# iyak/RNAelem

Hardware: AMD Instinct MI355X
Metric: train-iter seqs/sec (inside+outside) (higher is better)
Workload: dtype f64; 1 GPU; 10000 synthetic RNAs L=200, pattern ((.*.)), W=50 C=30 min_bpp=1e-4 T2004, x0 lambda=(1,1), one (fn,gr) eval per step; n_seq=10000, seq_len=200, pattern=((.*.)), bpp_filter=cached (computed once at load_batch, 0.1 s incl. plan), n_skipped=0

## Files before the change

rnaelem_amd/csrc/lin_fast.h:

```cpp
#pragma once
#include "lin_rules.h"
#include "plan_rules.h"

namespace elemdp {

#ifndef ELEMDP_UNARY2
#define ELEMDP_UNARY2 1
#endif

constexpr int kCellInD = 10;
constexpr int kCellOutD = 14;
enum : int { CF_POK = 1, CF_LOK = 2, CF_MOK = 4, CF_EOK = 8, CF_DO2 = 16, CF_DOM = 32, CF_CE = 64, CF_CP = 128,
             CF_UP = 64, CF_DOL = 128,
             CF_YL = 1 << 17, CF_YR = 1 << 18, CF_JLAST = 1 << 19,
             CF_USH = 20 };
ELEMDP_HD int fcol(int packed, int byte) { const int c = (packed >> (8 * byte)) & 0xff; return c == 0xff ? -1 : c; }

ELEMDP_HD double cell_in_fetch(const SeqView& q, int d, int i, int k) {
  const int c_here = q.cell(i, d), c_up = (i > 0 && d + 2 <= q.W) ? q.cell(i - 1, d + 2) : c_here;
  const int term = k < 2 ? XT_STACK : k < 4 ? XT_ML : k < 6 ? XT_CLOSE : XT_HP;
  return xw_cell(q, k & 1, term, k < 4 ? c_here : c_up);
}
ELEMDP_HD int cell_in_flags(const ModelView& m, const SeqView& q, int d, int i) {
  const int j = i + d;
// ... 255 lines not shown
  __builtin_amdgcn_sched_barrier(0);
#endif
  const double in1 = in.ldc(ST_1, d, i, c1o, lok && u1), in2 = in.ldc(ST_2, d, i, c2o, lok && u2), inL = LPOST ? 0. : in.ldc(ST_L, d, i, cLo, isloop && uL);
  const double r7 = out.ldc(ST_P, d, i, cPo, pok);
  double op2[kFR], opL[kFR];
  int eR[kFR];
#pragma unroll
  for (int u = 0; u < kFR; ++u) {
    eR[u] = P[4 + u];
    op2[u] = out.ldc(ST_2, dp1, i, fcol(eR[u], 0), u < nRR && do2);
    opL[u] = LPOST ? 0. : out.ldc(ST_L, dp1, i, fcol(eR[u], 1), u < nRR && doL && eR[u] < 0);
  }
#endif
  const double in2z = in2 * invZ, inLz = inL * invZ;
  const bool a2 = do2 && in2 != 0., aL = !LPOST && doL && inL != 0.;
#pragma unroll
  for (int u = 0; u < kFR; ++u)
    if (u < nRR && (a2 || aL)) {
      const int id = (eR[u] >> 16) & 0x7fff;
      const int enr = G[A.fe_r + 2 * id], fr = G[A.fe_r + 2 * id + 1];
      const double w = lin[A.lin_wr + 5 * id + br] * ((fr & 1) ? ews_r : 1.);
      const double t2 = a2 ? op2[u] * w : 0., tL = aL ? opL[u] * w : 0.;
      const double z = fma(t2, in2z, tL * inLz);
      if (SCANM && !fast_scan_stat<MODE, false, true>(sink, FS[id], i - 1, j, yl, yr, jlast, z)) continue;
      if (MODE != OUT_END && !no_prf && z != 0. && br) sink.en(enr + br, z);
      s2 += t2;
      sL += tL;
    }
  double H1 = ph[0], H2 = ph[CS], HP = ph[2 * CS], HL = LPOST ? 0. : ph[3 * CS];
  for (int r = 1; r < nrep; ++r) {
    H1 += ph[r * rstride]; H2 += ph[r * rstride + CS]; HP += ph[r * rstride + 2 * CS];
    if (!LPOST) HL += ph[r * rstride + 3 * CS];
  }
  const double o1 = (in1 != 0.) ? H1 : 0.;
  const double oB = lok ? (mok ? oM : 0.) + o1 : 0.;
  const double o2 = (in2 != 0.) ? o1 + s2 : 0.;
  if (lok && c2o >= 0) out.band[out.cidx(ST_2, d, i, c2o)] = o2;
  double oP = 0.;
  if (inP != 0.) {
    const double t3b = (o2 + H2) * cr[6 + kl], z = t3b * inPz;
    if (MODE == OUT_TRAIN && z != 0.) sink.eh(ehs, cr[13] * z);
    oP = oP1b + t3b + (HP + r7);
  }
  if (pok && cPo >= 0) out.band[out.cidx(ST_P, d, i, cPo)] = oP;
  if (LPOST) return oB;
  double oL = 0.;
  if (inL != 0.) {
    const double t6b = oE * cr[4 + kl], z = t6b * inLz;
    if (MODE == OUT_TRAIN && z != 0.) sink.eh(ehs, cr[11] * z);
    oL = t6b + sL + HL;
  }
  if (cLo >= 0) out.band[out.cidx(ST_L, d, i, cLo)] = oL;
  return oB;
}

ELEMDP_HD double loop_outside_seed_term(double oE, double inP, double inLo, double xw) { return oE * (inP * inLo) * xw; }

template <int kFR, class Sink>
ELEMDP_HD double loop_outside_entry(const int32_t* P, const int32_t* G, int fe_r, const double* wr, const double* parent, double inL,
                                    double HL, double oE, double xhp, double e_hp, bool doL, int br, double ews_r, double invZ, int ehs,
                                    bool no_prf, Sink& sink) {
  if (inL == 0.) return 0.;
  const int nRR = (P[0] >> 8) & 15;
  const double inLz = inL * invZ;
  double sL = 0.;
  if (doL) {
#pragma unroll
    for (int u = 0; u < kFR; ++u)
      if (u < nRR) {
        const int e = P[4 + u], c = fcol(e, 1), id = (e >> 16) & 0x7fff;
        const int enr = G[fe_r + 2 * id], fr = G[fe_r + 2 * id + 1];
        const double w = wr[5 * id + br] * ((fr & 1) ? ews_r : 1.);
        const double tL = (e < 0 && c >= 0) ? parent[c] * w : 0.;
        const double z = tL * inLz;
        if (!no_prf && z != 0. && br) sink.en(enr + br, z);
        sL += tL;
      }
  }
  const double t6b = oE * xhp, z = t6b * inLz;
  if (z != 0.) sink.eh(ehs, e_hp * z);
  return t6b + sL + HL;
}

}
```

rnaelem_amd/csrc/lin_kernels.hip:

```cpp
#include <hip/hip_runtime.h>

#include <algorithm>
#include <cstdio>
#include <cstdlib>
#include <type_traits>

#ifndef ELEMDP_KCI
#define ELEMDP_KCI 2
#endif
#ifndef ELEMDP_LB_IN
#define ELEMDP_LB_IN 4
#endif
#ifndef ELEMDP_LB_IN_FAST
#define ELEMDP_LB_IN_FAST 8
#endif
#ifndef ELEMDP_LB_CYK
#define ELEMDP_LB_CYK 8
#endif
#ifndef ELEMDP_LB_OUT6
#define ELEMDP_LB_OUT6 6
#endif
#ifndef ELEMDP_LB_OUT
#define ELEMDP_LB_OUT 4
#endif
// ... 1616 lines not shown
      }
    }
    hp[slot] = oB;
  }
  __syncthreads();
  if (!(a.dbg & 1) && !(a.dbg & 128) && !(ELEMDP_KO & 8)) {
    const int nA = A.n_ap;
    double* const en_keep = sink.en_;
    for (int w = tid; w < nc * nA; w += kBT) {
      const int c = div_rcp(w, a.rcp_nap), p = w - c * nA;
      if (ci(c) + d <= end_ys) continue;
      if (FAST) {
        const int32_t* PR = G + A.fpr_out + 8 * p;
        const int r0 = PR[0], r1 = PR[1];
        const int tg = (r0 >> 16) & 0xff;
        const bool w1 = pi.merged && (r0 & (4 << 24));
        const int i = ci(c), j = i + d, dmi = dm[c];
        const bool exists = dmi > 0 && dmi < d;
        const bool dead = MASK && exists && !((crfl[c] >> CF_USH) & UB_A);
        if (dead) {
          out.a(d, i, p) = 0.;
        } else if (exists) {
          const bool step = d + 1 <= W && j < L && v.q.unp[j];
          const int nr = step ? (r1 >> 20) & 15 : 0;
          const double a_in = in.a(d, i, p);
          int ce[kFastR];
          double op[kFastR];
#pragma unroll
          for (int u = 0; u < kFastR; ++u) {
            ce[u] = PR[5 + u];
            op[u] = out.lda(d + 1, i, u < nr ? ce[u] & 0xff : p, u < nr);
          }
          double acc = 0.;
          if (a_in != 0.) {
            acc = tg != 0xff ? hp[c * HD + tg] : 0.;
            const double inz = a_in * (w1 ? pi.invZs : pi.invZ);
            const int bj = step ? (int)v.q.seq[j] : 0;
            const double ewj = step ? v.q.ews[j] : 1.;
            double* en = l_en + (w1 ? nt : 0);
#pragma unroll
            for (int u = 0; u < kFastR; ++u)
              if (u < nr) {
                const int id = (ce[u] >> 8) & 0x7fff;
                const double term = op[u] * (v.m.lin[A.lin_wr + 5 * id + bj] * ((G[A.fe_r + 2 * id + 1] & 1) ? ewj : 1.));
                const double z = term * inz;
                if ((MODE == OUT_SCAN || MODE == OUT_END) &&
                    !fast_scan_stat<MODE, false, true>(sink, G[A.fs_out + id], i - 1, j, false, MODE == OUT_END && j == a.ys[v.n], L == j + 1, z))
                  continue;
                if (MODE != OUT_END && !v.m.no_prf && z != 0. && bj) atomicAdd(&en[G[A.fe_r + 2 * id] + bj], z);
                acc += term;
              }
          }
          out.a(d, i, p) = acc;
        }
        continue;
      }
      const int tgt = v.m.ints[A.ap_tgt + p];
      const bool w1 = pi.merged && v.m.ints[A.ap_t + p] == A.shadow;
      sink.en_ = l_en + (w1 ? nt : 0);
      LinOutCtx<LinSink> x{v.m, v.q, in, out, w1 ? pi.invZs : pi.invZ, sink, Constraint{MODE == OUT_END ? a.ys[v.n] : -1, -1, 0}};
      lin_outside_apair<MODE>(x, d, i0 + c, p, tgt >= 0 ? hp[c * HD + tgt] : 0.);
    }
    sink.en_ = en_keep;
  }
  pc.mark<11>();
  if (MODE == OUT_SCAN || MODE == OUT_END) {
    __syncthreads();
    const int p1 = (i0 + nc + d < L) ? i0 + nc + d : L;
    for (int t = tid; t <= p1 - pos_p0; t += kBT) {
      const double v0 = l_pos[t], v1 = l_pos[win + t];
      if (MODE == OUT_SCAN) {
        if (v0 != 0. && pos_p0 + t < L) atomicAdd(&a.pos_start[v.seq_base + pos_p0 + t], v0);
        if (v1 != 0. && pos_p0 + t < L) atomicAdd(&a.pos_inner[v.seq_base + pos_p0 + t], v1);
      } else if (v0 != 0.) {
        atomicAdd(&a.pos_end[v.pos_base + pos_p0 + t], v0);
      }
    }
  }
  if (MODE == OUT_TRAIN || MODE == OUT_SCAN) lflush(a, v, pi, sink, l_en0, kBT, (int)bx);
  pc.mark<12>();
  pc.finish();
}

constexpr int kSeedRows = 8, kSeedDiags = 17, kSeedCap = 256;
static size_t loop_seed_lds(const AutomatonLayout& A) {
  return sizeof(double) * ((size_t)kSeedRows * kSeedDiags * A.n_lane + 2 * kSeedCap) +
         sizeof(int32_t) * (kSeedRows * (kSeedDiags + 1) + kSeedRows + 1 + kLoopColsMax + 4 * kSeedCap + 2 * (size_t)A.n_quad);
}
__global__ __launch_bounds__(kBT) void k4_out_seed(LinArgs a) {
  extern __shared__ double lds[];
  LViews v(a.lay);
  make_lviews(a, blockIdx.y, v);
  if (v.row[4] != 0.) return;
  const AutomatonLayout& A = a.lay;
  const int tid = threadIdx.x, L = v.q.L, W = v.q.W;
  const int i0 = blockIdx.x * kSeedRows, d0 = blockIdx.z * kSeedDiags;
  if (d0 > W || i0 + d0 > L) return;
  const int nrow = (kSeedRows < L - i0 + 1) ? kSeedRows : L - i0 + 1, nd = (kSeedDiags < W - d0 + 1) ? kSeedDiags : W - d0 + 1;
  const int HD = A.n_lane, nq = A.n_quad, rs = v.out.rs[ST_L];
  double* acc = lds;
  double* s_xw = acc + kSeedRows * kSeedDiags * HD;
  int* offs = reinterpret_cast<int*>(s_xw + 2 * kSeedCap);
  int* pre = offs + kSeedRows * (kSeedDiags + 1);
  int* cmap = pre + kSeedRows + 1;
  int* s_row = cmap + kLoopColsMax;
  int* tq = s_row + 4 * kSeedCap;
  for (int t = tid; t < kSeedRows * kSeedDiags * HD; t += kBT) acc[t] = 0.;
  if (tid < kLoopColsMax) cmap[tid] = -1;
  __syncthreads();
  for (int k = tid; k < HD; k += kBT) {
    const int c = fcol(a.ints[A.fp_out + a.ints[A.f_live_out + k] * kFastW + 2], 2);
    if (c >= 0 && c < kLoopColsMax) cmap[c] = k;
  }
  const int32_t* G = v.m.big;
  const double* IB = v.in.band;
  const double* OB = v.out.band;
  const float rcp_nq = 1.0f / (float)(nq > 0 ? nq : 1);
  for (int role = 1; role <= 2; ++role) {
    const int32_t* off = role == 1 ? v.q.by_left_off : v.q.by_right_off;
    const LoopItem* items = role == 1 ? v.q.items_left : v.q.items_right;
    __syncthreads();
    for (int t = tid; t < nrow * (nd + 1); t += kBT) {
      const int r = t / (nd + 1), dd = t - r * (nd + 1), d = d0 + dd;
      offs[r * (kSeedDiags + 1) + dd] = nq > 0 ? off[v.q.cell(i0 + r, d > 0 ? d : 1)] : 0;
    }
    for (int t = tid; t < 2 * nq; t += kBT) tq[t] = G[A.fqc_out + role * 2 * nq + t];
    __syncthreads();
    if (tid == 0) {
      int n = 0;
      for (int r = 0; r < nrow; ++r) { pre[r] = n; n += offs[r * (kSeedDiags + 1) + nd] - offs[r * (kSeedDiags + 1)]; }
      pre[nrow] = n;
    }
    __syncthreads();
    const int n_rec = pre[nrow];
    for (int p0 = 0; p0 < n_rec; p0 += kSeedCap) {
      const int np = (kSeedCap < n_rec - p0) ? kSeedCap : n_rec - p0;
      for (int xs = tid; xs < np; xs += kBT) {
        const int x = p0 + xs;
        int r = 0;
        while (r + 1 < nrow && pre[r + 1] <= x) ++r;
        const int* ro = offs + r * (kSeedDiags + 1);
        const int n = ro[0] + (x - pre[r]);
        int dd = 0;
        while (dd + 1 < nd && ro[dd + 1] <= n) ++dd;
        const int i = i0 + r, d = d0 + dd;
        const bool on = i + d <= L && (v.q.ubits(i, d) & UB_L);
        const LoopItem it = items[n];
        s_row[xs] = (int)v.out.cidx(ST_E, it.j - it.i, it.i, 0);
        s_row[kSeedCap + xs] = (int)v.in.cidx(ST_P, it.l - it.k, it.k, 0);
        s_row[2 * kSeedCap + xs] = (int)(role == 1 ? v.in.cidx(ST_L, it.j - it.l, it.l, 0) : v.in.cidx(ST_L, it.k - it.i, it.i, 0));
        s_row[3 * kSeedCap + xs] = on ? (r * kSeedDiags + dd) * HD : -1;
        s_xw[xs] = lin_weight(v.m.lambda[0], it.tsc);
        s_xw[kSeedCap + xs] = lin_weight(v.m.lambda[1], it.tsc);
      }
      __syncthreads();
      for (int w = tid; w < np * nq; w += kBT) {
        const int xs = div_rcp(w, rcp_nq), t = w - xs * nq;
        const int cell = s_row[3 * kSeedCap + xs];
        const int qa = tq[2 * t], qb = tq[2 * t + 1];
        if (cell < 0 || (qb & (4 << 16))) continue;
        const double x0 = OB[(uint32_t)s_row[xs] + (qa & 0xff)], x1 = IB[(uint32_t)s_row[kSeedCap + xs] + ((qa >> 8) & 0xff)];
        const double x2 = IB[(uint32_t)s_row[2 * kSeedCap + xs] + ((qa >> 16) & 0xff)];
        const double term = loop_outside_seed_term(x0, x1, x2, s_xw[((qb >> 16) & 1) * kSeedCap + xs]);
        if (term != 0.) atomicAdd(&acc[cell + (qb & 0xffff)], term);
      }
      __syncthreads();
    }
  }
  __syncthreads();
  const int run = kSeedRows * rs;
  for (int t = tid; t < nd * run; t += kBT) {
    const int dd = t / run, e = t - dd * run, r = e / rs, c = e - r * rs, d = d0 + dd;
    if (i0 + r + d > L) continue;
    const int k = c < kLoopColsMax ? cmap[c] : -1;
    v.out.band[v.out.cidx(ST_L, d, i0, 0) + e] = k >= 0 ? acc[(r * kSeedDiags + dd) * HD + k] : 0.;
  }
}

static size_t loop_chain_lds(const AutomatonLayout& A) {
  return sizeof(double) * (2 * (size_t)kBT + 5 * (size_t)A.n_wr + 2 * (size_t)A.n_theta + 4) + sizeof(int32_t) * kLoopColsMax * (kLoopProgW + 1);
}
__global__ __launch_bounds__(kBT) void k4_out_loops(LinArgs a) {
  extern __shared__ double lds[];
  LViews v(a.lay);
  make_lviews(a, blockIdx.y, v);
  const LPass pi = lpass(a, v);
  if (pi.skip) return;
  const AutomatonLayout& A = a.lay;
  const int tid = threadIdx.x, L = v.q.L, W = v.q.W, nt = A.n_theta;
  const int rs = v.out.rs[ST_L], R = kBT / rs;
  const int i0 = blockIdx.x * R;
  if (i0 > L) return;
  double* cur = lds;
  double* prev = lds + kBT;
  double* wr = lds + 2 * kBT;
  double* l_en = wr + 5 * A.n_wr;
  int32_t* prog = reinterpret_cast<int32_t*>(l_en + 2 * nt + 4);
  int32_t* pst = prog + kLoopColsMax * kLoopProgW;
  for (int t = tid; t < kLoopColsMax * (kLoopProgW + 1); t += kBT) prog[t] = 0;
  for (int t = tid; t < 5 * A.n_wr; t += kBT) wr[t] = a.lin[A.lin_wr + t];
  for (int t = tid; t < 2 * nt + 4; t += kBT) l_en[t] = 0.;
  cur[tid] = 0.; prev[tid] = 0.;
  __syncthreads();
  for (int k = tid; k < A.n_lane; k += kBT) {
    const int s = a.ints[A.f_live_out + k];
    const int32_t* P = a.ints + A.fp_out + s * kFastW;
    const int c = fcol(P[2], 2);
    if (c >= 0 && c < kLoopColsMax) {
      for (int w = 0; w < kLoopProgW; ++w) prog[c * kLoopProgW + w] = P[w];
      pst[c] = s;
    }
  }
  __syncthreads();
  const int r = tid / rs, c = tid - r * rs, i = i0 + r;
  const int32_t* P = prog + (r < R ? c : 0) * kLoopProgW;
  const int w0 = P[0];
  const bool have = r < R && i <= L && (w0 & 1);
  const bool w1 = pi.merged && pst[r < R ? c : 0] == A.shadow;
  const int kl = (w0 >> 2) & 1, cEo = fcol(P[1], 1), ehs = v.m.lam_same ? 0 : kl;
  const double invZ = w1 ? pi.invZs : pi.invZ;
  LinSink sink;
  sink.world = w1 ? 1 : 0;
  sink.en_ = l_en + (w1 ? nt : 0);
  sink.eh0 = sink.eh1 = 0.;
  const int dmax = (W < L - i0) ? W : L - i0;
  auto cell_on = [&](int d) { return have && d >= 0 && i + d <= L && (v.q.ubits(i, d) & UB_L); };
  bool on_n = cell_on(dmax);
  double inL_n = on_n ? v.in.band[v.in.cidx(ST_L, dmax, i, c)] : 0., HL_n = on_n ? v.out.band[v.out.cidx(ST_L, dmax, i, c)] : 0.;
  for (int d = dmax; d >= 0; --d) {
    double oL = 0.;
    const bool on = on_n;
    const double inL = inL_n, HL = HL_n;
    on_n = cell_on(d - 1);
    inL_n = on_n ? v.in.band[v.in.cidx(ST_L, d - 1, i, c)] : 0.;
    HL_n = on_n ? v.out.band[v.out.cidx(ST_L, d - 1, i, c)] : 0.;
    if (on) {
      if (inL != 0.) {
        const int j = i + d;
        const bool eok = v.q.e_ok(i, d), doL = j < L && d + 1 <= W;
        const int c_up = eok ? v.q.cell(i - 1, d + 2) : v.q.cell(i, d);
        const double oE = (eok && cEo >= 0) ? v.out.band[v.out.cidx(ST_E, d, i, cEo)] : 0.;
        const double xhp = eok ? xw_cell(v.q, kl, XT_HP, c_up) : 0.;
        oL = loop_outside_entry<kFastR>(P, v.m.big, A.fe_r, wr, prev + r * rs, inL, HL, oE, xhp, v.q.e_hp[c_up], doL, j < L ? (int)v.q.seq[j] : 0,
                                        v.q.ews[j < L ? j : L], invZ, ehs, v.m.no_prf != 0, sink);
      }
    }
    cur[tid] = oL;
    __syncthreads();
    double* x = cur; cur = prev; prev = x;
  }
  lflush(a, v, pi, sink, l_en, kBT, (int)blockIdx.x);
}

__global__ __launch_bounds__(kThreads) void k4_combine(LinArgs a, int G) {
  const int g = blockIdx.x;
  if (g >= G) return;
  const int n = a.grp[g];
  double* row = a.seq_out + (size_t)n * a.out_stride;
  if (row[4] != 0.) return;
  const double* zs = a.zs + (size_t)g * 4;
  const int nt = a.lay.n_theta;
  if (a.det) {
    const double* dr = a.det_rows + (size_t)n * a.det_nslot * a.out_stride;
    for (int t = 6 + threadIdx.x; t < 6 + 2 * nt + 4; t += kThreads) {
      double acc = 0.;
      for (int k = 0; k < a.det_nslot; ++k) acc += dr[(size_t)k * a.out_stride + t];
      row[t] = acc;
    }
    __syncthreads();
  }
  const bool positive = a.plans[n].positive != 0;
  const double pa = zs[1] / zs[0], pn = zs[2] / zs[0];
  for (int t = threadIdx.x; t < nt + 2; t += kThreads) {
    double* A = (t < nt) ? &row[6 + t] : &row[6 + 2 * nt + (t - nt)];
    double* B = (t < nt) ? &row[6 + nt + t] : &row[6 + 2 * nt + 2 + (t - nt)];
    const double va = *A, vb = *B;
    if (a.schedule == 1) {
      const double full = pa * va + pn * vb;
      if (a.lik_ratio && !positive) { *A = va; *B = full; }
      else { *A = full; *B = positive ? va : vb; }
    } else if (a.lik_ratio && !positive) {
      *A = vb; *B = va;
    }
  }
}

__device__ __forceinline__ unsigned long long cyk_key(double v) {
  const long long b = __double_as_longlong(v + 0.);
  return (unsigned long long)(b >= 0 ? b : (b ^ 0x7fffffffffffffffLL)) ^ 0x8000000000000000ULL;
}
__device__ __forceinline__ double cyk_unkey(unsigned long long k) {
  const long long b = (long long)(k ^ 0x8000000000000000ULL);
  return __longlong_as_double(b >= 0 ? b : (b ^ 0x7fffffffffffffffLL));
}

__global__ __launch_bounds__(kThreads) void k5_cyk_serial(LinArgs a) {
  __shared__ AutomatonLayout s_lay;
  stage_layout(a, &s_lay, kThreads);
  unsigned bx, by;
  swizzled_block(bx, by);
  LViews v(s_lay);
  make_lviews(a, by, v);
  __syncthreads();
  const int S = a.lay.S, d = a.d;
  if (d > v.q.W) return;
  const int t = bx * kThreads + threadIdx.x;
  if (t >= (v.q.L - d + 1) * S) return;
  const int i = t / S, s = t - i * S;
  TraceView R;
  R.ext = nullptr;
  const Constraint c{a.ys[v.n], a.ye[v.n], 1};
  cyk_target(v.m, v.q, v.in, R, c, d, i, s);
}

template <bool BIG, int KOWN>
__global__ __launch_bounds__(kBT, KOWN <= 2 ? ELEMDP_LB_CYK : 6) void k5_cyk(LinArgs a) {
  extern __shared__ double lds[];

  unsigned bx, by;
  swizzled_block(bx, by);
  LViews v(a.lay);
  make_lviews(a, by, v);
  const AutomatonLayout& A = a.lay;
  const int S = a.lay.S, d = a.d, cpb = a.cpb, tid = threadIdx.x;
  if (d > v.q.W) return;
  const int ncell = v.q.L - d + 1, i0 = bx * cpb;
  if (i0 >= ncell) return;
  const int nc = (cpb < ncell - i0) ? cpb : ncell - i0;
  const int NL = A.n_lane;
  const int CS = cpb * NL;
  const double NEG = ELEMDP_NEG_INF;
  unsigned long long* kb = reinterpret_cast<unsigned long long*>(lds);
  unsigned long long* ke = kb + CS;
  double* st1 = lds + 2 * CS;
// ... 279 lines not shown
    case K4_GENERIC: hipLaunchKernelGGL((k4_in<false, CON>), grid, dim3(kBT), lds, st, a); break;
  }
}
template <int MODE>
static void launch_k4_out(const LinArgs& a, dim3 grid, size_t lds, bool fast, bool big, hipStream_t st) {
  if (MODE == OUT_TRAIN && fast && a.loop_post) {
    const bool l = a.p.blocks != nullptr;
    switch (k4_form(a, lds, 6, fast, big)) {
      case K4_FP2_WAVES:
        if (l) hipLaunchKernelGGL((k4_out<OUT_TRAIN, true, true, 2, true, true, true>), grid, dim3(kBT), lds, st, a);
        else hipLaunchKernelGGL((k4_out<OUT_TRAIN, true, true, 2, true, false, true>), grid, dim3(kBT), lds, st, a);
        return;
      case K4_FP2:
        if (l) hipLaunchKernelGGL((k4_out<OUT_TRAIN, true, true, 2, false, true, true>), grid, dim3(kBT), lds, st, a);
        else hipLaunchKernelGGL((k4_out<OUT_TRAIN, true, true, 2, false, false, true>), grid, dim3(kBT), lds, st, a);
        return;
      default:
        if (l) hipLaunchKernelGGL((k4_out<OUT_TRAIN, true, true, kFastP, false, true, true>), grid, dim3(kBT), lds, st, a);
        else hipLaunchKernelGGL((k4_out<OUT_TRAIN, true, true, kFastP, false, false, true>), grid, dim3(kBT), lds, st, a);
        return;
    }
  }
  if (MODE == OUT_TRAIN && fast && a.p.blocks) {
    switch (k4_form(a, lds, 6, fast, big)) {
      case K4_FP2_WAVES: hipLaunchKernelGGL((k4_out<OUT_TRAIN, true, true, 2, true, true>), grid, dim3(kBT), lds, st, a); return;
      case K4_FP2: hipLaunchKernelGGL((k4_out<OUT_TRAIN, true, true, 2, false, true>), grid, dim3(kBT), lds, st, a); return;
      default: hipLaunchKernelGGL((k4_out<OUT_TRAIN, true, true, kFastP, false, true>), grid, dim3(kBT), lds, st, a); return;
    }
  }
  switch (k4_form(a, lds, 6, fast, big)) {
    case K4_FP2_WAVES: hipLaunchKernelGGL((k4_out<MODE, true, true, 2, true>), grid, dim3(kBT), lds, st, a); break;
    case K4_FP2: hipLaunchKernelGGL((k4_out<MODE, true, true, 2>), grid, dim3(kBT), lds, st, a); break;
    case K4_FAST: hipLaunchKernelGGL((k4_out<MODE, true, true>), grid, dim3(kBT), lds, st, a); break;
    case K4_STAGED: hipLaunchKernelGGL((k4_out<MODE, true>), grid, dim3(kBT), lds, st, a); break;
    case K4_GENERIC: hipLaunchKernelGGL((k4_out<MODE, false>), grid, dim3(kBT), lds, st, a); break;
  }
}
template <>
void launch_k4_out<OUT_NONE>(const LinArgs& a, dim3 grid, size_t lds, bool, bool, hipStream_t st) {
  hipLaunchKernelGGL((k4_out<OUT_NONE, true>), grid, dim3(kBT), lds, st, a);
}

struct GroupGeom {
  LinArgs a;
  bool big, fast;
  int hd, win;
  size_t lds_in, lds_out;
  bool stage_ext;
  size_t lds_ext_in;
  int ext_nt;
};
static bool geometry_fast(const LinArgs& a) {
  return a.fast && a.n_stage >= a.lay.n_ints && a.lay.fp_ok && !(a.dbg & 16) && a.lay.lin_total <= 2048;
}
int lin_train_cpb(const LinArgs& full) {
  return geometry_fast(full) ? std::min(kBT / std::max(full.lay.n_lane, 1), ELEMDP_CPB_MAX) : 0;
}
int lin_live_span_max() { return kLiveSpanMax; }
bool lin_loop_prepass_ok(const AutomatonLayout& A, const int32_t* ints, int min_span) {
  const bool say = getenv("ELEMDP_PLAN_DEBUG") != nullptr;
  if (!A.fp_ok || A.tab_rs[ST_L] < 1 || A.tab_rs[ST_L] > kLoopColsMax || loop_prepass_lds(A) > 64 * 1024) {
    if (say) fprintf(stderr, "loop pre-pass: not for this automaton (fp_ok %d, L row of %d columns)\n", A.fp_ok, A.tab_rs[ST_L]);
    return false;
  }
  auto col = [](int packed, int byte) { const int c = (packed >> (8 * byte)) & 0xff; return c == 0xff ? -1 : c; };
  unsigned seen = 0;
  for (int k = 0; k < A.n_lane; ++k) {
    const int32_t* P = ints + A.fp_in + ints[A.f_live_in + k] * kFastW;
    const int c = col(P[2], 2);
    if (c >= 0) {
      if (c >= A.tab_rs[ST_L] || ((seen >> c) & 1u)) { if (say) fprintf(stderr, "loop pre-pass: not for this automaton (column %d of lane %d)\n", c, k); return false; }
      seen |= 1u << c;
      continue;
    }
    if (!(P[0] & 1) || col(P[1], 1) < 0) continue;
    const int nR = (P[0] >> 8) & 15;
    bool zero = !(P[0] & 2) || min_span > 2;
    for (int u = 0; u < nR && u < kFastR; ++u) zero = zero && col(P[4 + u], 0) < 0;
    if (!zero) { if (say) fprintf(stderr, "loop pre-pass: not for this automaton (lane %d: a loop state with an E column, no L column and an L value)\n", k); return false; }
  }
  return true;
}
static bool loop_outside_lds_ok(const AutomatonLayout& A) {
  return A.tab_rs[ST_L] >= 1 && A.tab_rs[ST_L] <= kLoopColsMax && kBT / A.tab_rs[ST_L] >= 1 && loop_seed_lds(A) <= 64 * 1024 && loop_chain_lds(A) <= 64 * 1024;
}
bool lin_loop_outside_ok(const AutomatonLayout& A, const int32_t* ints) {
  const bool say = getenv("ELEMDP_PLAN_DEBUG") != nullptr;
  if (!A.fp_ok || !loop_outside_lds_ok(A)) {
    if (say) fprintf(stderr, "L kernels behind the outside sweep: not for this automaton (fp_ok %d, L row of %d columns, LDS %zu / %zu)\n", A.fp_ok, A.tab_rs[ST_L], loop_seed_lds(A), loop_chain_lds(A));
    return false;
  }
  auto col = [](int packed, int byte) { const int c = (packed >> (8 * byte)) & 0xff; return c == 0xff ? -1 : c; };
  unsigned seen = 0;
  for (int k = 0; k < A.n_lane; ++k) {
    const int s = ints[A.f_live_out + k];
    const int c = col(ints[A.fp_out + s * kFastW + 2], 2), ci = col(ints[A.fp_in + s * kFastW + 2], 2);
    if (c != ci || (c >= 0 && (c >= A.tab_rs[ST_L] || ((seen >> c) & 1u)))) {
      if (say) fprintf(stderr, "L kernels behind the outside sweep: not for this automaton (state %d: L column %d outside, %d inside)\n", s, c, ci);
      return false;
    }
    if (c >= 0) seen |= 1u << c;
  }
  return true;
}
static GroupGeom group_geometry(const LinArgs& full, int G, int Lmax, int Wmax, bool scan) {
  GroupGeom g;
  LinArgs& a = g.a;
  a = full;
  const int S = a.lay.S, nt = a.lay.n_theta;
  a.cpb = std::min(kBT / S, ELEMDP_CPB_MAX);
  a.wmax = Wmax;
  a.ext_ring = G <= 1024 ? 1 : 0;
  a.lmax = Lmax;
  if (scan) { a.schedule = 0; a.pass = 0; a.scan = 1; a.det = 0; }
  g.big = a.n_stage >= a.lay.n_ints;
  const bool fast = g.fast = geometry_fast(a);
  a.fast = fast ? 1 : 0;
  if (fast) a.cpb = std::min(kBT / std::max(a.lay.n_lane, 1), ELEMDP_CPB_MAX);
  a.n_lin = fast ? a.lay.lin_total : kLinEth + nt;
  const int NW = a.det ? kBT / 64 : 1;
  g.hd = fast ? a.lay.n_lane : S;
  set_rcps(a, fast);
  if (scan || !fast || a.det || !a.p.useful || !a.p.blocks || !a.blk_grid || a.live_span < a.cpb) { a.p.blocks = nullptr; a.blk_grid = nullptr; a.live_span = 0; }
  if (scan || !fast || !a.p.useful) a.loop_pre = 0;
  if (a.loop_pre && a.p.blocks && (!a.p.blocks_in || !a.blk_grid_in)) a.loop_pre = 0;
  if (scan || !fast || !a.p.useful || a.det) a.loop_post = 0;
  if (a.loop_post && a.p.blocks && (!a.p.blocks_in || !a.blk_grid_in)) a.loop_post = 0;
  if (a.loop_post && !loop_outside_lds_ok(a.lay)) a.loop_post = 0;
  const int sp = a.live_span > a.cpb ? a.live_span : a.cpb;
  g.win = sp + Wmax + 3;
  g.lds_in = block_lds(2 * a.cpb * g.hd + kRecIn, a.cpb, a.n_lin, g.win, fast ? a.lay.fb_in_n : staged_ints(a.lay, a.n_stage, 0), 0, fast ? kCellInD : 0, sp).total;
  g.lds_out = block_lds(out_doubles(a.cpb * g.hd, nt, g.win, NW, scan), a.cpb, a.n_lin, g.win, fast ? a.lay.fb_out_n : staged_ints(a.lay, a.n_stage, 1), 3 * a.cpb, fast ? kCellOutD : 0, sp).total;
  g.stage_ext = Lmax <= 2048 && a.nword_max <= 8192;
  g.lds_ext_in = g.stage_ext ? (size_t)ext_lds((a.ext_ring ? ext_ring_doubles(0, Wmax, S, kLinEth + nt, Lmax, a.nword_max, a.n_stage) : 0), kLinEth + nt, Lmax, a.nword_max, a.n_stage).total : 0;
  g.ext_nt = (a.ext_block == kExtBlock && a.ext_ring && a.lay.n_active <= 128 && !(a.dbg & 8192)) ? 128 * kExtBlock : 128;
  return g;
}
static unsigned band_blocks(LinArgs& a, int ncell, bool train) {
  const int n = (ncell + a.cpb - 1) / a.cpb;
  if (!train || !a.blk_grid || !a.p.blocks) return (unsigned)n;
  if (a.blk_grid[a.d] < 0) { a.p.blocks = nullptr; return (unsigned)n; }
  return (unsigned)std::max(1, std::min(n, a.blk_grid[a.d]));
}
template <bool CON>
static void inside_sweeps(GroupGeom& g, int G, int Lmax, int Wmax, bool bands, hipStream_t st) {
  LinArgs& a = g.a;
  const bool pre = !CON && bands && g.fast && a.loop_pre;
  LinArgs ai = a;
  if (!pre) ai.loop_pre = 0;
  if (pre) {
    if (a.p.blocks) { ai.p.blocks = a.p.blocks_in; ai.blk_grid = a.blk_grid_in; }
    hipLaunchKernelGGL(k4_in_loops, dim3((Lmax + kLoopLanes) / kLoopLanes, G), dim3(kLoopLanes), loop_prepass_lds(a.lay), st, ai);
  }
  if (bands)
    for (int d = pre ? a.in_d0 : 0; d <= Wmax; ++d) {
      const int ncell = Lmax - d + 1;
      if (ncell <= 0) break;
      LinArgs ad = ai;
      ad.d = d;
      const unsigned gx = band_blocks(ad, ncell, !CON);
      launch_k4_in<CON>(ad, dim3(gx, G), g.lds_in, g.fast, g.big, st);
    }
  if (g.stage_ext) hipLaunchKernelGGL((k4_in_ext<true, CON>), dim3(G), dim3(g.ext_nt), g.lds_ext_in, st, a);
  else hipLaunchKernelGGL((k4_in_ext<false, CON>), dim3(G), dim3(128), 0, st, a);
}
template <int MODE>
static void outside_bands(GroupGeom& g, int G, int Lmax, int Wmax, hipStream_t st) {
  LinArgs& a = g.a;
  hipLaunchKernelGGL(k4_r7, dim3(((Lmax + 1) * (Wmax + 1) + kThreads - 1) / kThreads, G), dim3(kThreads), 0, st, a);
  const bool post = MODE == OUT_TRAIN && g.fast && a.loop_post;
  LinArgs ao = a;
  if (!post) ao.loop_post = 0;
  if (post && a.p.blocks) { ao.p.blocks = a.p.blocks_in; ao.blk_grid = a.blk_grid_in; }
  for (int d = Wmax; d >= (post ? a.in_d0 : 0); --d) {
    const int ncell = Lmax - d + 1;
    if (ncell <= 0) continue;
    LinArgs ad = ao;
    ad.d = d;
    const unsigned gx = band_blocks(ad, ncell, MODE == OUT_TRAIN);
    launch_k4_out<MODE>(ad, dim3(gx, G), g.lds_out, g.fast, g.big, st);
  }
  if (post) {
    hipLaunchKernelGGL(k4_out_seed, dim3((Lmax + kSeedRows) / kSeedRows, G, (Wmax + kSeedDiags) / kSeedDiags), dim3(kBT), loop_seed_lds(a.lay), st, a);
    const int rows = kBT / a.lay.tab_rs[ST_L];
    hipLaunchKernelGGL(k4_out_loops, dim3((Lmax + rows) / rows, G), dim3(kBT), loop_chain_lds(a.lay), st, a);
  }
}
template <bool CON, int MODE>
static void scan_sweeps(GroupGeom& g, int G, int Lmax, int Wmax, hipStream_t st) {
  const LinArgs& a = g.a;
  const int S = a.lay.S, nt = a.lay.n_theta;
  const size_t lds_ext_out = g.stage_ext ? (size_t)ext_lds(2 * nt + 4 + (a.ext_ring ? ext_ring_doubles(2 * nt + 4, Wmax, S, kLinEth + nt, Lmax, a.nword_max, a.n_stage) : 0), kLinEth + nt, Lmax, a.nword_max, a.n_stage).total : sizeof(double) * (2 * nt + 4);
  inside_sweeps<CON>(g, G, Lmax, Wmax, true, st);
  if (g.stage_ext) hipLaunchKernelGGL((k4_out_ext<MODE, true>), dim3(G), dim3(g.ext_nt), lds_ext_out, st, a);
  else hipLaunchKernelGGL((k4_out_ext<MODE, false>), dim3(G), dim3(128), lds_ext_out, st, a);
  outside_bands<MODE>(g, G, Lmax, Wmax, st);
}

hipError_t launch_lin_scan_group(const LinArgs& full, int G, int Lmax, int Wmax, ScanPass pass, hipStream_t st) {
  if (G <= 0) return hipSuccess;
  GroupGeom g = group_geometry(full, G, Lmax, Wmax, true);
  const LinArgs& a = g.a;
  if (getenv("ELEMDP_LDS_DEBUG") && pass == SCAN_PASS_START) fprintf(stderr, "scan group: G %d cpb %d S %d nt %d fast %d n_lin %d fast blob in/out %d/%d ints win %d lds k4_in %zu k4_out %zu\n", G, a.cpb, a.lay.S, a.lay.n_theta, (int)g.fast, a.n_lin, a.lay.fb_in_n, a.lay.fb_out_n, g.win, g.lds_in, g.lds_out);
  if (pass == SCAN_PASS_INSIDE) {
    inside_sweeps<false>(g, G, Lmax, Wmax, true, st);
  } else if (pass == SCAN_PASS_START) {
    scan_sweeps<false, OUT_SCAN>(g, G, Lmax, Wmax, st);
    hipLaunchKernelGGL(k5_pick<0>, dim3((G + 63) / 64), dim3(64), 0, st, a, G);
  } else {
    scan_sweeps<true, OUT_END>(g, G, Lmax, Wmax, st);
    hipLaunchKernelGGL(k5_pick<1>, dim3((G + 63) / 64), dim3(64), 0, st, a, G);
  }
  return hipGetLastError();
}

hipError_t launch_lin_group(const LinArgs& full, int G, int Lmax, int Wmax, bool first_pass_only, hipStream_t st) {
  if (G <= 0) return hipSuccess;
  GroupGeom g = group_geometry(full, G, Lmax, Wmax, false);
  const LinArgs& a = g.a;
  const int S = a.lay.S, nt = a.lay.n_theta;
  inside_sweeps<false>(g, G, Lmax, Wmax, !a.no_rss, st);
  const int n_pass = (a.schedule == 1 || first_pass_only) ? 1 : 2;
  const bool combine = (a.schedule == 1 || a.lik_ratio || a.det) && !first_pass_only;
  if (getenv("ELEMDP_LDS_DEBUG")) {
    const bool stats = !(g.big && (a.dbg & 16));
    fprintf(stderr, "lin group: G %d cpb %d fast %d n_lin %d staged ints in/out %d/%d lds k4_in %zu k4_out %zu fp_max_p %d forms k4_in %s k4_out %s stage_ext %d ext_nt %d ext_ring %d n_pass %d combine %d\n", G, a.cpb, (int)g.fast, a.n_lin, staged_ints(a.lay, a.n_stage, 0), staged_ints(a.lay, a.n_stage, 1), g.lds_in, g.lds_out, a.lay.fp_max_p,
            a.no_rss ? "none" : kK4FormName[k4_form(a, g.lds_in, 8, g.fast, g.big)], a.no_rss ? "none" : !stats ? "nostat" : kK4FormName[k4_form(a, g.lds_out, 6, g.fast, g.big)],
            (int)g.stage_ext, g.stage_ext ? g.ext_nt : 128, a.ext_ring, n_pass, (int)combine);
    fprintf(stderr, "lin group: loop_prepass %d loop_outside %d (k4_out_seed lds %zu, k4_out_loops lds %zu)\n", a.loop_pre, a.loop_post, loop_seed_lds(a.lay), loop_chain_lds(a.lay));
  }
  for (int pass = 0; pass < n_pass; ++pass) {
    GroupGeom gp = g;
    LinArgs& b = gp.a;
    b.pass = pass;
    const int n_stat = ext_stat_doubles(nt, b.det);
    if (g.stage_ext) hipLaunchKernelGGL((k4_out_ext<OUT_TRAIN, true>), dim3(G), dim3(b.det ? 128 : g.ext_nt), (size_t)ext_lds(n_stat + (b.ext_ring ? ext_ring_doubles(n_stat, Wmax, S, kLinEth + nt, Lmax, b.nword_max, b.n_stage) : 0), kLinEth + nt, Lmax, b.nword_max, b.n_stage).total, st, b);
    else hipLaunchKernelGGL((k4_out_ext<OUT_TRAIN, false>), dim3(G), dim3(128), sizeof(double) * n_stat, st, b);
    if (b.no_rss) continue;
    if (g.big && (b.dbg & 16)) outside_bands<OUT_NONE>(gp, G, Lmax, Wmax, st);
    else outside_bands<OUT_TRAIN>(gp, G, Lmax, Wmax, st);
  }
  if (combine) hipLaunchKernelGGL(k4_combine, dim3(G), dim3(kThreads), 0, st, a, G);
  return hipGetLastError();
}

}
```

Measured before the change: 49080 seq/s.

## Fuse loop-outside seed and chain kernels into one row-tiled kernel

```diff
diff --git a/rnaelem_amd/csrc/lin_fast.h b/rnaelem_amd/csrc/lin_fast.h
--- a/rnaelem_amd/csrc/lin_fast.h
+++ b/rnaelem_amd/csrc/lin_fast.h
@@ -361,4 +361,29 @@
   return t6b + sL + HL;
 }
 
-}
+template <class Sink>
+ELEMDP_HD double loop_outside_cell(double inL, double oE, double xhp, double e_hp, double invZ, int ehs, Sink& sink) {
+  const double t6b = oE * xhp, z = t6b * (inL * invZ);
+  if (z != 0.) sink.eh(ehs, e_hp * z);
+  return t6b;
+}
+template <int kFR, class Sink>
+ELEMDP_HD double loop_outside_chain(const int32_t* P, const int* enr, const int* fr, const double* wr, const double* parent, double inL,
+                                    int br, double ews_r, double invZ, bool no_prf, Sink& sink) {
+  const int nRR = (P[0] >> 8) & 15;
+  const double inLz = inL * invZ;
+  double sL = 0.;
+#pragma unroll
+  for (int u = 0; u < kFR; ++u)
+    if (u < nRR) {
+      const int e = P[4 + u], c = fcol(e, 1), id = (e >> 16) & 0x7fff;
+      const double w = wr[5 * id + br] * ((fr[u] & 1) ? ews_r : 1.);
+      const double tL = (e < 0 && c >= 0) ? parent[c] * w : 0.;
+      const double z = tL * inLz;
+      if (!no_prf && z != 0. && br) sink.en(enr[u] + br, z);
+      sL += tL;
+    }
+  return sL;
+}
+
+}
diff --git a/rnaelem_amd/csrc/lin_kernels.hip b/rnaelem_amd/csrc/lin_kernels.hip
--- a/rnaelem_amd/csrc/lin_kernels.hip
+++ b/rnaelem_amd/csrc/lin_kernels.hip
@@ -1722,174 +1722,228 @@
   pc.finish();
 }
 
-constexpr int kSeedRows = 8, kSeedDiags = 17, kSeedCap = 256;
-static size_t loop_seed_lds(const AutomatonLayout& A) {
-  return sizeof(double) * ((size_t)kSeedRows * kSeedDiags * A.n_lane + 2 * kSeedCap) +
-         sizeof(int32_t) * (kSeedRows * (kSeedDiags + 1) + kSeedRows + 1 + kLoopColsMax + 4 * kSeedCap + 2 * (size_t)A.n_quad);
-}
-__global__ __launch_bounds__(kBT) void k4_out_seed(LinArgs a) {
+constexpr int kRowsT = 8, kRowsMax = 32, kSeedCap = 256, kSeedBatch = 2;
+static_assert(2 * kRowsMax <= 64, "the runs of a tile are scanned by one wave");
+__host__ __device__ inline int loop_rows_r(int rs) { const int r = kBT / (rs > 0 ? rs : 1); return r < kRowsMax ? r : kRowsMax; }
+static size_t loop_rows_lds(const AutomatonLayout& A) {
+  const size_t rs = A.tab_rs[ST_L], R = loop_rows_r(A.tab_rs[ST_L]);
+  return sizeof(double) * (R * (kRowsT + 1) * rs + 2 * kSeedCap + (R + kRowsT) + 5 * (size_t)A.n_wr + 2 * (size_t)A.n_theta + 4) +
+         sizeof(int32_t) * (2 * R * (kRowsT + 1) + 2 * R + 1 + 4 * kSeedCap + 4 * (size_t)A.n_quad + (size_t)A.n_lane + kLoopColsMax * (kLoopProgW + 1) + (R + kRowsT));
+}
+__global__ __launch_bounds__(kBT) void k4_out_lrows(LinArgs a) {
   extern __shared__ double lds[];
+  unsigned bx, by;
+  swizzled_block(bx, by);
   LViews v(a.lay);
-  make_lviews(a, blockIdx.y, v);
-  if (v.row[4] != 0.) return;
+  make_lviews(a, by, v);
+  const LPass pi = lpass(a, v);
+  if (pi.skip) return;
   const AutomatonLayout& A = a.lay;
-  const int tid = threadIdx.x, L = v.q.L, W = v.q.W;
-  const int i0 = blockIdx.x * kSeedRows, d0 = blockIdx.z * kSeedDiags;
-  if (d0 > W || i0 + d0 > L) return;
-  const int nrow = (kSeedRows < L - i0 + 1) ? kSeedRows : L - i0 + 1, nd = (kSeedDiags < W - d0 + 1) ? kSeedDiags : W - d0 + 1;
-  const int HD = A.n_lane, nq = A.n_quad, rs = v.out.rs[ST_L];
+  const int tid = threadIdx.x, L = v.q.L, W = v.q.W, nt = A.n_theta, nq = A.n_quad, HD = A.n_lane;
+  const int rs = v.out.rs[ST_L], R = loop_rows_r(rs), TS = (kRowsT + 1) * rs;
+  const int i0 = bx * R;
+  if (i0 > L) return;
+  const int nrow = (R < L - i0 + 1) ? R : L - i0 + 1, nrr = 2 * nrow;
   double* acc = lds;
-  double* s_xw = acc + kSeedRows * kSeedDiags * HD;
-  int* offs = reinterpret_cast<int*>(s_xw + 2 * kSeedCap);
-  int* pre = offs + kSeedRows * (kSeedDiags + 1);
-  int* cmap = pre + kSeedRows + 1;
-  int* s_row = cmap + kLoopColsMax;
+  double* s_xw = acc + R * TS;
+  double* s_ew = s_xw + 2 * kSeedCap;
+  double* wr = s_ew + R + kRowsT;
+  double* l_en = wr + 5 * A.n_wr;
+  int* offs = reinterpret_cast<int*>(l_en + 2 * nt + 4);
+  int* pre = offs + 2 * R * (kRowsT + 1);
+  int* s_row = pre + 2 * R + 1;
   int* tq = s_row + 4 * kSeedCap;
-  for (int t = tid; t < kSeedRows * kSeedDiags * HD; t += kBT) acc[t] = 0.;
-  if (tid < kLoopColsMax) cmap[tid] = -1;
+  int* lcol = tq + 4 * nq;
+  int32_t* prog = lcol + HD;
+  int32_t* pst = prog + kLoopColsMax * kLoopProgW;
+  int* s_b = pst + kLoopColsMax;
+  const int32_t* G = v.m.big;
+  for (int t = tid; t < kLoopColsMax * (kLoopProgW + 1); t += kBT) prog[t] = 0;
+  for (int t = tid; t < 5 * A.n_wr; t += kBT) wr[t] = a.lin[A.lin_wr + t];
+  for (int t = tid; t < 2 * nt + 4; t += kBT) l_en[t] = 0.;
+  for (int t = tid; t < 4 * nq; t += kBT) tq[t] = G[A.fqc_out + 2 * nq + t];
   __syncthreads();
   for (int k = tid; k < HD; k += kBT) {
-    const int c = fcol(a.ints[A.fp_out + a.ints[A.f_live_out + k] * kFastW + 2], 2);
-    if (c >= 0 && c < kLoopColsMax) cmap[c] = k;
-  }
-  const int32_t* G = v.m.big;
+    const int s = a.ints[A.f_live_out + k];
+    const int32_t* P = a.ints + A.fp_out + s * kFastW;
+    const int c = fcol(P[2], 2);
+    lcol[k] = (c >= 0 && c < rs) ? c : -1;
+    if (c >= 0 && c < kLoopColsMax) {
+      for (int w = 0; w < kLoopProgW; ++w) prog[c * kLoopProgW + w] = P[w];
+      pst[c] = s;
+    }
+  }
+  __syncthreads();
+  const int r = tid / rs, c = tid - r * rs, i = i0 + r;
+  const bool lane = r < R;
+  const int32_t* P = prog + (lane ? c : 0) * kLoopProgW;
+  const int w0 = P[0];
+  const bool have = lane && i <= L && (w0 & 1);
+  const bool w1 = pi.merged && pst[lane ? c : 0] == A.shadow;
+  const int kl = (w0 >> 2) & 1, cEo = fcol(P[1], 1), ehs = v.m.lam_same ? 0 : kl;
+  const double invZ = w1 ? pi.invZs : pi.invZ;
+  int enr[kFastR], fr[kFastR];
+#pragma unroll
+  for (int u = 0; u < kFastR; ++u) {
+    const bool on = u < ((w0 >> 8) & 15);
+    const int id = on ? (P[4 + u] >> 16) & 0x7fff : 0;
+    enr[u] = on ? G[A.fe_r + 2 * id] : 0;
+    fr[u] = on ? G[A.fe_r + 2 * id + 1] : 0;
+  }
+  LinSink sink;
+  sink.world = w1 ? 1 : 0;
+  sink.en_ = l_en + (w1 ? nt : 0);
+  sink.eh0 = sink.eh1 = 0.;
+  double* const row_e = acc + (lane ? r * TS + c : 0);
+  const float rcp_nq = 1.0f / (float)(nq > 0 ? nq : 1);
   const double* IB = v.in.band;
   const double* OB = v.out.band;
-  const float rcp_nq = 1.0f / (float)(nq > 0 ? nq : 1);
-  for (int role = 1; role <= 2; ++role) {
-    const int32_t* off = role == 1 ? v.q.by_left_off : v.q.by_right_off;
-    const LoopItem* items = role == 1 ? v.q.items_left : v.q.items_right;
+  const int dmax = (W < L - i0) ? W : L - i0;
+  double carry = 0.;
+  for (int dhi = dmax; dhi >= 0; dhi -= kRowsT) {
+    const int d0 = dhi >= kRowsT ? dhi - kRowsT + 1 : 0, nd = dhi - d0 + 1;
+    double inL[kRowsT], t6[kRowsT];
+    {
+      int ub[kRowsT];
+      uint32_t pw[kRowsT];
+#pragma unroll
+      for (int dd = 0; dd < kRowsT; ++dd) {
+        const int d = d0 + dd;
+        const bool in = have && dd < nd && i + d <= L;
+        const bool up = in && i > 0 && d + 2 <= W && i + d + 1 <= L;
+        ub[dd] = v.q.ubits(in ? i : 0, in ? d : 0);
+        ub[dd] = in ? ub[dd] : 0;
+        pw[dd] = v.q.okbits[up ? (uint32_t)v.q.cell(i - 1, d + 2) >> 5 : 0u];
+        pw[dd] = up ? pw[dd] : 0u;
+      }
+#pragma unroll
+      for (int dd = 0; dd < kRowsT; ++dd) {
+        const int d = d0 + dd, c_up = v.q.cell(i - 1, d + 2);
+        const bool on = (ub[dd] & UB_L) != 0, eok = on && ((pw[dd] >> (c_up & 31)) & 1u);
+        inL[dd] = v.in.ldc(ST_L, d, i, c, on);
+        const double oE = v.out.ldc(ST_E, d, i, cEo, eok), xhp = xw_cell(v.q, kl, XT_HP, eok ? c_up : 0), ehp = v.q.e_hp[eok ? c_up : 0];
+        t6[dd] = 0.;
+        if (eok && inL[dd] != 0.) t6[dd] = loop_outside_cell(inL[dd], oE, xhp, ehp, invZ, ehs, sink);
+      }
+    }
+    if (lane) {
+#pragma unroll
+      for (int dd = 0; dd < kRowsT; ++dd) row_e[dd * rs] = dd == nd ? carry : t6[dd];
+      row_e[kRowsT * rs] = carry;
+    }
+    {
+      constexpr int kOffU = (2 * kRowsMax * (kRowsT + 1) + kBT - 1) / kBT;
+      int ov[kOffU], os[kOffU];
+#pragma unroll
+      for (int u = 0; u < kOffU; ++u) {
+        const int t = tid + u * kBT;
+        const bool ok = t < nrr * (nd + 1) && nq > 0;
+        const int rr = ok ? div_small(t, nd + 1) : 0, dd = ok ? t - rr * (nd + 1) : 0, role = rr >= nrow, d = d0 + dd;
+        const int32_t* off = role ? v.q.by_right_off : v.q.by_left_off;
+        os[u] = t < nrr * (nd + 1) ? rr * (kRowsT + 1) + dd : -1;
+        ov[u] = off[ok ? v.q.cell(i0 + rr - role * nrow, d > 0 ? d : 1) : 0];
+        ov[u] = ok ? ov[u] : 0;
+      }
+      int lo = 0, hi = 0;
+      if (tid < 64) {
+        const bool ok = tid < nrr && nq > 0;
+        const int role = tid >= nrow, ri = i0 + tid - role * nrow;
+        const int32_t* off = role ? v.q.by_right_off : v.q.by_left_off;
+        lo = off[ok ? v.q.cell(ri, d0 > 0 ? d0 : 1) : 0];
+        hi = off[ok ? v.q.cell(ri, d0 + nd) : 0];
+        lo = ok ? lo : 0;
+        hi = ok ? hi : 0;
+      }
+      int jb = 0;
+      double jw = 0.;
+      if (tid < nrow + nd) {
+        const int j = i0 + d0 + tid;
+        jb = j < L ? (int)v.q.seq[j] : 0;
+        jw = v.q.ews[j < L ? j : L];
+      }
+#pragma unroll
+      for (int u = 0; u < kOffU; ++u)
+        if (os[u] >= 0) offs[os[u]] = ov[u];
+      if (tid < 64) {
+        int n = hi - lo;
+#pragma unroll
+        for (int sft = 1; sft < 64; sft <<= 1) {
+          const int up = __shfl_up(n, sft);
+          if (tid >= sft) n += up;
+        }
+        if (tid < nrr) pre[tid + 1] = n;
+        if (tid == 0) pre[0] = 0;
+      }
+      if (tid < nrow + nd) { s_b[tid] = jb; s_ew[tid] = jw; }
+    }
     __syncthreads();
-    for (int t = tid; t < nrow * (nd + 1); t += kBT) {
-      const int r = t / (nd + 1), dd = t - r * (nd + 1), d = d0 + dd;
-      offs[r * (kSeedDiags + 1) + dd] = nq > 0 ? off[v.q.cell(i0 + r, d > 0 ? d : 1)] : 0;
-    }
-    for (int t = tid; t < 2 * nq; t += kBT) tq[t] = G[A.fqc_out + role * 2 * nq + t];
-    __syncthreads();
-    if (tid == 0) {
-      int n = 0;
-      for (int r = 0; r < nrow; ++r) { pre[r] = n; n += offs[r * (kSeedDiags + 1) + nd] - offs[r * (kSeedDiags + 1)]; }
-      pre[nrow] = n;
-    }
-    __syncthreads();
-    const int n_rec = pre[nrow];
+    const int n_rec = pre[nrr];
     for (int p0 = 0; p0 < n_rec; p0 += kSeedCap) {
       const int np = (kSeedCap < n_rec - p0) ? kSeedCap : n_rec - p0;
       for (int xs = tid; xs < np; xs += kBT) {
         const int x = p0 + xs;
-        int r = 0;
-        while (r + 1 < nrow && pre[r + 1] <= x) ++r;
-        const int* ro = offs + r * (kSeedDiags + 1);
-        const int n = ro[0] + (x - pre[r]);
+        int rr = 0;
+        while (rr + 1 < nrr && pre[rr + 1] <= x) ++rr;
+        const int* ro = offs + rr * (kRowsT + 1);
+        const int n = ro[0] + (x - pre[rr]);
         int dd = 0;
         while (dd + 1 < nd && ro[dd + 1] <= n) ++dd;
-        const int i = i0 + r, d = d0 + dd;
-        const bool on = i + d <= L && (v.q.ubits(i, d) & UB_L);
-        const LoopItem it = items[n];
+        const int role = rr >= nrow, rw = rr - role * nrow, ri = i0 + rw, d = d0 + dd;
+        const bool on = ri + d <= L && (v.q.ubits(ri, d) & UB_L);
+        const LoopItem it = (role ? v.q.items_right : v.q.items_left)[n];
         s_row[xs] = (int)v.out.cidx(ST_E, it.j - it.i, it.i, 0);
         s_row[kSeedCap + xs] = (int)v.in.cidx(ST_P, it.l - it.k, it.k, 0);
-        s_row[2 * kSeedCap + xs] = (int)(role == 1 ? v.in.cidx(ST_L, it.j - it.l, it.l, 0) : v.in.cidx(ST_L, it.k - it.i, it.i, 0));
-        s_row[3 * kSeedCap + xs] = on ? (r * kSeedDiags + dd) * HD : -1;
+        s_row[2 * kSeedCap + xs] = (int)(role ? v.in.cidx(ST_L, it.k - it.i, it.i, 0) : v.in.cidx(ST_L, it.j - it.l, it.l, 0));
+        s_row[3 * kSeedCap + xs] = on ? 2 * (rw * TS + dd * rs) + role : -1;
         s_xw[xs] = lin_weight(v.m.lambda[0], it.tsc);
         s_xw[kSeedCap + xs] = lin_weight(v.m.lambda[1], it.tsc);
       }
       __syncthreads();
-      for (int w = tid; w < np * nq; w += kBT) {
-        const int xs = div_rcp(w, rcp_nq), t = w - xs * nq;
-        const int cell = s_row[3 * kSeedCap + xs];
-        const int qa = tq[2 * t], qb = tq[2 * t + 1];
-        if (cell < 0 || (qb & (4 << 16))) continue;
-        const double x0 = OB[(uint32_t)s_row[xs] + (qa & 0xff)], x1 = IB[(uint32_t)s_row[kSeedCap + xs] + ((qa >> 8) & 0xff)];
-        const double x2 = IB[(uint32_t)s_row[2 * kSeedCap + xs] + ((qa >> 16) & 0xff)];
-        const double term = loop_outside_seed_term(x0, x1, x2, s_xw[((qb >> 16) & 1) * kSeedCap + xs]);
-        if (term != 0.) atomicAdd(&acc[cell + (qb & 0xffff)], term);
+      for (int wb = tid; wb < np * nq; wb += kSeedBatch * kBT) {
+        double x0[kSeedBatch], x1[kSeedBatch], x2[kSeedBatch], xw[kSeedBatch];
+        int dst[kSeedBatch];
+#pragma unroll
+        for (int u = 0; u < kSeedBatch; ++u) {
+          const int w = wb + u * kBT;
+          const bool in = w < np * nq;
+          const int xs = in ? div_rcp(w, rcp_nq) : 0, t = in ? w - xs * nq : 0;
+          const int cell = s_row[3 * kSeedCap + xs];
+          const int32_t* q2 = tq + (cell & 1) * 2 * nq + 2 * t;
+          const int qa = q2[0], qb = q2[1], col = lcol[qb & 0xffff];
+          const bool ok = in && cell >= 0 && col >= 0 && !(qb & (4 << 16));
+          dst[u] = ok ? (cell >> 1) + col : -1;
+          x0[u] = OB[ok ? (uint32_t)s_row[xs] + (qa & 0xff) : 0u];
+          x1[u] = IB[ok ? (uint32_t)s_row[kSeedCap + xs] + ((qa >> 8) & 0xff) : 0u];
+          x2[u] = IB[ok ? (uint32_t)s_row[2 * kSeedCap + xs] + ((qa >> 16) & 0xff) : 0u];
+          xw[u] = s_xw[((qb >> 16) & 1) * kSeedCap + xs];
+        }
+#pragma unroll
+        for (int u = 0; u < kSeedBatch; ++u)
+          if (dst[u] >= 0) {
+            const double term = loop_outside_seed_term(x0[u], x1[u], x2[u], xw[u]);
+            if (term != 0.) atomicAdd(&acc[dst[u]], term);
+          }
       }
       __syncthreads();
     }
-  }
-  __syncthreads();
-  const int run = kSeedRows * rs;
-  for (int t = tid; t < nd * run; t += kBT) {
-    const int dd = t / run, e = t - dd * run, r = e / rs, c = e - r * rs, d = d0 + dd;
-    if (i0 + r + d > L) continue;
-    const int k = c < kLoopColsMax ? cmap[c] : -1;
-    v.out.band[v.out.cidx(ST_L, d, i0, 0) + e] = k >= 0 ? acc[(r * kSeedDiags + dd) * HD + k] : 0.;
-  }
-}
-
-static size_t loop_chain_lds(const AutomatonLayout& A) {
-  return sizeof(double) * (2 * (size_t)kBT + 5 * (size_t)A.n_wr + 2 * (size_t)A.n_theta + 4) + sizeof(int32_t) * kLoopColsMax * (kLoopProgW + 1);
-}
-__global__ __launch_bounds__(kBT) void k4_out_loops(LinArgs a) {
-  extern __shared__ double lds[];
-  LViews v(a.lay);
-  make_lviews(a, blockIdx.y, v);
-  const LPass pi = lpass(a, v);
-  if (pi.skip) return;
-  const AutomatonLayout& A = a.lay;
-  const int tid = threadIdx.x, L = v.q.L, W = v.q.W, nt = A.n_theta;
-  const int rs = v.out.rs[ST_L], R = kBT / rs;
-  const int i0 = blockIdx.x * R;
-  if (i0 > L) return;
-  double* cur = lds;
-  double* prev = lds + kBT;
-  double* wr = lds + 2 * kBT;
-  double* l_en = wr + 5 * A.n_wr;
-  int32_t* prog = reinterpret_cast<int32_t*>(l_en + 2 * nt + 4);
-  int32_t* pst = prog + kLoopColsMax * kLoopProgW;
-  for (int t = tid; t < kLoopColsMax * (kLoopProgW + 1); t += kBT) prog[t] = 0;
-  for (int t = tid; t < 5 * A.n_wr; t += kBT) wr[t] = a.lin[A.lin_wr + t];
-  for (int t = tid; t < 2 * nt + 4; t += kBT) l_en[t] = 0.;
-  cur[tid] = 0.; prev[tid] = 0.;
-  __syncthreads();
-  for (int k = tid; k < A.n_lane; k += kBT) {
-    const int s = a.ints[A.f_live_out + k];
-    const int32_t* P = a.ints + A.fp_out + s * kFastW;
-    const int c = fcol(P[2], 2);
-    if (c >= 0 && c < kLoopColsMax) {
-      for (int w = 0; w < kLoopProgW; ++w) prog[c * kLoopProgW + w] = P[w];
-      pst[c] = s;
-    }
-  }
-  __syncthreads();
-  const int r = tid / rs, c = tid - r * rs, i = i0 + r;
-  const int32_t* P = prog + (r < R ? c : 0) * kLoopProgW;
-  const int w0 = P[0];
-  const bool have = r < R && i <= L && (w0 & 1);
-  const bool w1 = pi.merged && pst[r < R ? c : 0] == A.shadow;
-  const int kl = (w0 >> 2) & 1, cEo = fcol(P[1], 1), ehs = v.m.lam_same ? 0 : kl;
-  const double invZ = w1 ? pi.invZs : pi.invZ;
-  LinSink sink;
-  sink.world = w1 ? 1 : 0;
-  sink.en_ = l_en + (w1 ? nt : 0);
-  sink.eh0 = sink.eh1 = 0.;
-  const int dmax = (W < L - i0) ? W : L - i0;
-  auto cell_on = [&](int d) { return have && d >= 0 && i + d <= L && (v.q.ubits(i, d) & UB_L); };
-  bool on_n = cell_on(dmax);
-  double inL_n = on_n ? v.in.band[v.in.cidx(ST_L, dmax, i, c)] : 0., HL_n = on_n ? v.out.band[v.out.cidx(ST_L, dmax, i, c)] : 0.;
-  for (int d = dmax; d >= 0; --d) {
-    double oL = 0.;
-    const bool on = on_n;
-    const double inL = inL_n, HL = HL_n;
-    on_n = cell_on(d - 1);
-    inL_n = on_n ? v.in.band[v.in.cidx(ST_L, d - 1, i, c)] : 0.;
-    HL_n = on_n ? v.out.band[v.out.cidx(ST_L, d - 1, i, c)] : 0.;
-    if (on) {
-      if (inL != 0.) {
-        const int j = i + d;
-        const bool eok = v.q.e_ok(i, d), doL = j < L && d + 1 <= W;
-        const int c_up = eok ? v.q.cell(i - 1, d + 2) : v.q.cell(i, d);
-        const double oE = (eok && cEo >= 0) ? v.out.band[v.out.cidx(ST_E, d, i, cEo)] : 0.;
-        const double xhp = eok ? xw_cell(v.q, kl, XT_HP, c_up) : 0.;
-        oL = loop_outside_entry<kFastR>(P, v.m.big, A.fe_r, wr, prev + r * rs, inL, HL, oE, xhp, v.q.e_hp[c_up], doL, j < L ? (int)v.q.seq[j] : 0,
-                                        v.q.ews[j < L ? j : L], invZ, ehs, v.m.no_prf != 0, sink);
-      }
-    }
-    cur[tid] = oL;
-    __syncthreads();
-    double* x = cur; cur = prev; prev = x;
-  }
-  lflush(a, v, pi, sink, l_en, kBT, (int)blockIdx.x);
+    double oL = carry;
+#pragma unroll
+    for (int dd = kRowsT - 1; dd >= 0; --dd) {
+      if (dd >= nd) continue;
+      oL = 0.;
+      if (inL[dd] != 0.) {
+        const int d = d0 + dd, j = i + d;
+        double sL = 0.;
+        if (j < L && d + 1 <= W)
+          sL = loop_outside_chain<kFastR>(P, enr, fr, wr, row_e + (dd + 1) * rs - c, inL[dd], s_b[r + dd], s_ew[r + dd], invZ, v.m.no_prf != 0, sink);
+        oL = row_e[dd * rs] + sL;
+      }
+      if (lane) row_e[dd * rs] = oL;
+      __syncthreads();
+    }
+    carry = oL;
+  }
+  lflush(a, v, pi, sink, l_en, kBT, (int)bx);
 }
 
 __global__ __launch_bounds__(kThreads) void k4_combine(LinArgs a, int G) {
@@ -2335,12 +2389,12 @@
   return true;
 }
 static bool loop_outside_lds_ok(const AutomatonLayout& A) {
-  return A.tab_rs[ST_L] >= 1 && A.tab_rs[ST_L] <= kLoopColsMax && kBT / A.tab_rs[ST_L] >= 1 && loop_seed_lds(A) <= 64 * 1024 && loop_chain_lds(A) <= 64 * 1024;
+  return A.tab_rs[ST_L] >= 1 && A.tab_rs[ST_L] <= kLoopColsMax && A.tab_rs[ST_L] <= kBT && loop_rows_lds(A) <= 64 * 1024;
 }
 bool lin_loop_outside_ok(const AutomatonLayout& A, const int32_t* ints) {
   const bool say = getenv("ELEMDP_PLAN_DEBUG") != nullptr;
   if (!A.fp_ok || !loop_outside_lds_ok(A)) {
-    if (say) fprintf(stderr, "L kernels behind the outside sweep: not for this automaton (fp_ok %d, L row of %d columns, LDS %zu / %zu)\n", A.fp_ok, A.tab_rs[ST_L], loop_seed_lds(A), loop_chain_lds(A));
+    if (say) fprintf(stderr, "L kernel behind the outside sweep: not for this automaton (fp_ok %d, L row of %d columns, LDS %zu)\n", A.fp_ok, A.tab_rs[ST_L], loop_rows_lds(A));
     return false;
   }
   auto col = [](int packed, int byte) { const int c = (packed >> (8 * byte)) & 0xff; return c == 0xff ? -1 : c; };
@@ -2434,9 +2488,8 @@
     launch_k4_out<MODE>(ad, dim3(gx, G), g.lds_out, g.fast, g.big, st);
   }
   if (post) {
-    hipLaunchKernelGGL(k4_out_seed, dim3((Lmax + kSeedRows) / kSeedRows, G, (Wmax + kSeedDiags) / kSeedDiags), dim3(kBT), loop_seed_lds(a.lay), st, a);
-    const int rows = kBT / a.lay.tab_rs[ST_L];
-    hipLaunchKernelGGL(k4_out_loops, dim3((Lmax + rows) / rows, G), dim3(kBT), loop_chain_lds(a.lay), st, a);
+    const int rows = loop_rows_r(a.lay.tab_rs[ST_L]);
+    hipLaunchKernelGGL(k4_out_lrows, dim3((Lmax + rows) / rows, G), dim3(kBT), loop_rows_lds(a.lay), st, a);
   }
 }
 template <bool CON, int MODE>
@@ -2480,7 +2533,7 @@
     fprintf(stderr, "lin group: G %d cpb %d fast %d n_lin %d staged ints in/out %d/%d lds k4_in %zu k4_out %zu fp_max_p %d forms k4_in %s k4_out %s stage_ext %d ext_nt %d ext_ring %d n_pass %d combine %d\n", G, a.cpb, (int)g.fast, a.n_lin, staged_ints(a.lay, a.n_stage, 0), staged_ints(a.lay, a.n_stage, 1), g.lds_in, g.lds_out, a.lay.fp_max_p,
             a.no_rss ? "none" : kK4FormName[k4_form(a, g.lds_in, 8, g.fast, g.big)], a.no_rss ? "none" : !stats ? "nostat" : kK4FormName[k4_form(a, g.lds_out, 6, g.fast, g.big)],
             (int)g.stage_ext, g.stage_ext ? g.ext_nt : 128, a.ext_ring, n_pass, (int)combine);
-    fprintf(stderr, "lin group: loop_prepass %d loop_outside %d (k4_out_seed lds %zu, k4_out_loops lds %zu)\n", a.loop_pre, a.loop_post, loop_seed_lds(a.lay), loop_chain_lds(a.lay));
+    fprintf(stderr, "lin group: loop_prepass %d loop_outside %d (k4_out_lrows lds %zu, %d rows x %d diagonals)\n", a.loop_pre, a.loop_post, loop_rows_lds(a.lay), loop_rows_r(a.lay.tab_rs[ST_L]), kRowsT);
   }
   for (int pass = 0; pass < n_pass; ++pass) {
     GroupGeom gp = g;
```

Result: faster. 50630 seq/s (median of 6 runs) (+3.2%).
